# ch4r10t33r/zigz

Hardware: AMD Instinct MI355X
Metric: trace steps/sec proved (BabyBear, 2^20 RV64I trace) (higher is better)
Workload: dtype u32

## Files before the change

zigz_amd/csrc/host_hash.hpp:

```cpp
#pragma once
#include <stddef.h>
#include <stdint.h>

namespace zk {

class Sha3_256 {
  public:
    Sha3_256() { reset(); }
    void reset();
    void update(const uint8_t *data, size_t len);
    void update_le64(uint64_t v);
    void digest_copy(uint8_t out[32]) const;
    void finalize(uint8_t out[32]);
    uint64_t *raw_state() { return st_; }
    size_t *raw_pos() { return &pos_; }

  private:
    uint64_t st_[25];
    size_t pos_;
};

class Transcript {
  public:
    void append_bytes(const uint8_t *d, size_t n) { h_.update(d, n); }
    void append_field(uint64_t canonical) { h_.update_le64(canonical); }
    uint64_t challenge();
    void append_tagged_counter(const uint8_t *tag, size_t tag_len, uint64_t start, uint64_t count);

  private:
    Sha3_256 h_;
};

void sha3_256(const uint8_t *data, size_t len, uint8_t out[32]);
const char *host_keccak_impl();
void host_keccak_permute(uint64_t st[25], int which);
void sha256(const uint8_t *data, size_t len, uint8_t out[32]);

void host_sponge_servers(int n);
bool host_sponge_batching();
bool host_sponge_absorb_tagged(uint64_t st[25], size_t *pos, const uint8_t *tag, size_t tag_len, uint64_t start, uint64_t count);
void host_keccak_permute_x8(uint64_t st[25][8]);

}
```

zigz_amd/csrc/host_sponge_batch.cpp:

```cpp
#include <immintrin.h>
#include <stdint.h>
#include <stdlib.h>
#include <string.h>

#include <algorithm>
#include <atomic>
#include <condition_variable>
#include <deque>
#include <mutex>
#include <thread>
#include <vector>

#include "field.hpp"
#include "host_hash.hpp"

namespace zk {

bool cpu_has_avx512f();

namespace {

constexpr int SLOTS = 8;
constexpr size_t RATE = 136;

const uint64_t RC8[24] = {
    0x0000000000000001ull, 0x0000000000008082ull, 0x800000000000808aull, 0x8000000080008000ull, 0x000000000000808bull,
    0x0000000080000001ull, 0x8000000080008081ull, 0x8000000000008009ull, 0x000000000000008aull, 0x0000000000000088ull,
    0x0000000080008009ull, 0x000000008000000aull, 0x000000008000808bull, 0x800000000000008bull, 0x8000000000008089ull,
    0x8000000000008003ull, 0x8000000000008002ull, 0x8000000000000080ull, 0x000000000000800aull, 0x800000008000000aull,
    0x8000000080008081ull, 0x8000000000008080ull, 0x0000000080000001ull, 0x8000000080008008ull};

__attribute__((target("avx512f"))) void keccak_f1600_x8(uint64_t st[25][SLOTS]) {
#define X8_X3(a, b, c) _mm512_ternarylogic_epi64((a), (b), (c), 0x96)
#define X8_CHI(a, b, c) _mm512_ternarylogic_epi64((a), (b), (c), 0xD2)
#define X8_ROL(a, n) _mm512_rol_epi64((a), (n))
#define X8_B(n, a, cm, rp) X8_ROL(X8_X3(a, cm, rp), n)
#define X8_LD(i) _mm512_load_si512(st[i])
    __m512i a0 = X8_LD(0), a1 = X8_LD(1), a2 = X8_LD(2), a3 = X8_LD(3), a4 = X8_LD(4), a5 = X8_LD(5), a6 = X8_LD(6), a7 = X8_LD(7);
    __m512i a8 = X8_LD(8), a9 = X8_LD(9), a10 = X8_LD(10), a11 = X8_LD(11), a12 = X8_LD(12), a13 = X8_LD(13), a14 = X8_LD(14);
    __m512i a15 = X8_LD(15), a16 = X8_LD(16), a17 = X8_LD(17), a18 = X8_LD(18), a19 = X8_LD(19), a20 = X8_LD(20), a21 = X8_LD(21);
    __m512i a22 = X8_LD(22), a23 = X8_LD(23), a24 = X8_LD(24);
#pragma unroll 2
    for (int r = 0; r < 24; r++) {
        const __m512i c0 = X8_X3(X8_X3(a0, a5, a10), a15, a20), c1 = X8_X3(X8_X3(a1, a6, a11), a16, a21);
        const __m512i c2 = X8_X3(X8_X3(a2, a7, a12), a17, a22), c3 = X8_X3(X8_X3(a3, a8, a13), a18, a23);
        const __m512i c4 = X8_X3(X8_X3(a4, a9, a14), a19, a24);
        const __m512i r0 = X8_ROL(c0, 1), r1 = X8_ROL(c1, 1), r2 = X8_ROL(c2, 1), r3 = X8_ROL(c3, 1), r4 = X8_ROL(c4, 1);
        const __m512i b00 = X8_X3(a0, c4, r1);
        const __m512i b10 = X8_B(1, a1, c0, r2), b20 = X8_B(62, a2, c1, r3), b05 = X8_B(28, a3, c2, r4), b15 = X8_B(27, a4, c3, r0);
        const __m512i b16 = X8_B(36, a5, c4, r1), b01 = X8_B(44, a6, c0, r2), b11 = X8_B(6, a7, c1, r3), b21 = X8_B(55, a8, c2, r4);
        const __m512i b06 = X8_B(20, a9, c3, r0), b07 = X8_B(3, a10, c4, r1), b17 = X8_B(10, a11, c0, r2), b02 = X8_B(43, a12, c1, r3);
        const __m512i b12 = X8_B(25, a13, c2, r4), b22 = X8_B(39, a14, c3, r0), b23 = X8_B(41, a15, c4, r1), b08 = X8_B(45, a16, c0, r2);
        const __m512i b18 = X8_B(15, a17, c1, r3), b03 = X8_B(21, a18, c2, r4), b13 = X8_B(8, a19, c3, r0), b14 = X8_B(18, a20, c4, r1);
        const __m512i b24 = X8_B(2, a21, c0, r2), b09 = X8_B(61, a22, c1, r3), b19 = X8_B(56, a23, c2, r4), b04 = X8_B(14, a24, c3, r0);
        a0 = _mm512_xor_si512(X8_CHI(b00, b01, b02), _mm512_set1_epi64((long long)RC8[r]));
        a1 = X8_CHI(b01, b02, b03); a2 = X8_CHI(b02, b03, b04); a3 = X8_CHI(b03, b04, b00); a4 = X8_CHI(b04, b00, b01);
        a5 = X8_CHI(b05, b06, b07); a6 = X8_CHI(b06, b07, b08); a7 = X8_CHI(b07, b08, b09); a8 = X8_CHI(b08, b09, b05);
        a9 = X8_CHI(b09, b05, b06); a10 = X8_CHI(b10, b11, b12); a11 = X8_CHI(b11, b12, b13); a12 = X8_CHI(b12, b13, b14);
        a13 = X8_CHI(b13, b14, b10); a14 = X8_CHI(b14, b10, b11); a15 = X8_CHI(b15, b16, b17); a16 = X8_CHI(b16, b17, b18);
        a17 = X8_CHI(b17, b18, b19); a18 = X8_CHI(b18, b19, b15); a19 = X8_CHI(b19, b15, b16); a20 = X8_CHI(b20, b21, b22);
        a21 = X8_CHI(b21, b22, b23); a22 = X8_CHI(b22, b23, b24); a23 = X8_CHI(b23, b24, b20); a24 = X8_CHI(b24, b20, b21);
    }
#define X8_ST(i, v) _mm512_store_si512(st[i], (v))
    X8_ST(0, a0); X8_ST(1, a1); X8_ST(2, a2); X8_ST(3, a3); X8_ST(4, a4); X8_ST(5, a5); X8_ST(6, a6); X8_ST(7, a7); X8_ST(8, a8);
    X8_ST(9, a9); X8_ST(10, a10); X8_ST(11, a11); X8_ST(12, a12); X8_ST(13, a13); X8_ST(14, a14); X8_ST(15, a15); X8_ST(16, a16);
    X8_ST(17, a17); X8_ST(18, a18); X8_ST(19, a19); X8_ST(20, a20); X8_ST(21, a21); X8_ST(22, a22); X8_ST(23, a23); X8_ST(24, a24);
}

struct Job {
    uint64_t *st;
    size_t *pos;
    const uint8_t *tag;
    size_t tag_len;
    uint64_t start, count;
    std::mutex m;
    std::condition_variable cv;
    bool done = false;
};

struct Stream {
    static constexpr size_t CHUNK_RECORDS = 272;
    Job *job = nullptr;
    uint64_t v = 0, left = 0;
    size_t rec = 0, rd = 0, wr = 0;
    uint8_t tmpl[32];
    std::vector<uint8_t> buf;

    void open(Job *j) {
        job = j;
        rec = j->tag_len + 8;
        v = j->start % (uint64_t)P;
        left = j->count;
        rd = wr = 0;
        memset(tmpl, 0, sizeof(tmpl));
        memcpy(tmpl, j->tag, j->tag_len < 24 ? j->tag_len : 24);
        buf.resize(CHUNK_RECORDS * rec + RATE + 64);
    }
    size_t avail() const { return wr - rd; }
    bool exhausted() const { return left == 0 && rd == wr; }
    void fill() {
        if (avail() >= RATE || left == 0) return;
        if (rd) {
            memmove(buf.data(), buf.data() + rd, wr - rd);
            wr -= rd;
            rd = 0;
        }
        size_t m = (buf.size() - wr - 32) / rec;
        if (m > left) m = (size_t)left;
        uint8_t *q = buf.data() + wr;
        const size_t tl = job->tag_len;
        if (tl <= 24) {
            for (size_t k = 0; k < m; k++, q += rec) {
                memcpy(q, tmpl, 32);
                memcpy(q + tl, &v, 8);
                if (++v == (uint64_t)P) v = 0;
            }
        } else {
            for (size_t k = 0; k < m; k++, q += rec) {
                memcpy(q, job->tag, tl);
                memcpy(q + tl, &v, 8);
                if (++v == (uint64_t)P) v = 0;
            }
        }
        wr += m * rec;
        left -= m;
    }
};

class Service {
  public:
    ~Service() { resize(0); }

    void resize(int n) {
        std::unique_lock<std::mutex> lk(m_);
        if (n < 0) n = 0;
        if (n > 0 && !cpu_has_avx512f()) n = 0;
        if ((int)threads_.size() == n) return;
        enabled_.store(false, std::memory_order_release);
        stop_ = true;
        cv_.notify_all();
        std::vector<std::thread> old;
        old.swap(threads_);
        lk.unlock();
        for (auto &t : old) t.join();
        lk.lock();
        stop_ = false;
        for (int i = 0; i < n; i++) threads_.emplace_back([this] { serve(); });
        enabled_.store(n > 0, std::memory_order_release);
    }
    bool enabled() const { return enabled_.load(std::memory_order_acquire); }

    bool run(Job &j) {
        {
            std::lock_guard<std::mutex> lk(m_);
            if (threads_.empty() || stop_) return false;
            queue_.push_back(&j);
            pending_.fetch_add(1, std::memory_order_release);
        }
        cv_.notify_one();
        std::unique_lock<std::mutex> lk(j.m);
        j.cv.wait(lk, [&] { return j.done; });
        return true;
    }

  private:
    void serve() {
        alignas(64) uint64_t S[25][SLOTS];
        memset(S, 0, sizeof(S));
        Stream slot[SLOTS];
        size_t pos[SLOTS] = {0};
        int active = 0;
        for (;;) {
            if (active == 0 || (active < SLOTS && pending_.load(std::memory_order_acquire) > 0)) {
                std::unique_lock<std::mutex> lk(m_);
                if (active == 0) cv_.wait(lk, [&] { return stop_ || !queue_.empty(); });
                if (stop_ && active == 0 && queue_.empty()) return;
                for (int s = 0; s < SLOTS && !queue_.empty(); s++) {
                    if (slot[s].job) continue;
                    Job *j = queue_.front();
                    queue_.pop_front();
                    pending_.fetch_sub(1, std::memory_order_relaxed);
                    slot[s].open(j);
                    pos[s] = *j->pos;
                    for (int w = 0; w < 25; w++) S[w][s] = j->st[w];
                    active++;
                }
            }
            if (active == 1 && pending_.load(std::memory_order_acquire) == 0) {
                int s = 0;
                while (!slot[s].job) s++;
                Stream &st = slot[s];
                if (pos[s] == 0) {
                    uint64_t one[25];
                    for (int w = 0; w < 25; w++) one[w] = S[w][s];
                    for (int k = 0; k < 64; k++) {
                        st.fill();
                        if (st.avail() < RATE) break;
                        const uint8_t *src = st.buf.data() + st.rd;
                        for (int w = 0; w < 17; w++) {
                            uint64_t x;
                            memcpy(&x, src + 8 * w, 8);
                            one[w] ^= x;
                        }
                        st.rd += RATE;
                        host_keccak_permute(one, 0);
                    }
                    for (int w = 0; w < 25; w++) S[w][s] = one[w];
                }
            }
            bool permute = false;
            for (int s = 0; s < SLOTS; s++) {
                Stream &st = slot[s];
                if (!st.job) continue;
                st.fill();
                const size_t need = RATE - pos[s];
                size_t n = st.avail() < need ? st.avail() : need;
                const uint8_t *src = st.buf.data() + st.rd;
                if (pos[s] == 0 && n == RATE) {
                    for (int w = 0; w < 17; w++) {
                        uint64_t x;
                        memcpy(&x, src + 8 * w, 8);
                        S[w][s] ^= x;
                    }
                } else if (n) {
                    uint8_t blk[RATE] = {0};
                    memcpy(blk + pos[s], src, n);
                    for (int w = 0; w < 17; w++) {
                        uint64_t x;
                        memcpy(&x, blk + 8 * w, 8);
                        S[w][s] ^= x;
                    }
                }
                st.rd += n;
                pos[s] += n;
                if (pos[s] == RATE) {
                    pos[s] = 0;
                    permute = true;
                } else {
                    retire(S, s, slot, pos);
                    active--;
                }
            }
            if (permute) keccak_f1600_x8(S);
            for (int s = 0; s < SLOTS; s++)
                if (slot[s].job && slot[s].exhausted() && pos[s] == 0) {
                    retire(S, s, slot, pos);
                    active--;
                }
        }
    }

    static void retire(uint64_t S[25][SLOTS], int s, Stream *slot, size_t *pos) {
        Job *j = slot[s].job;
        for (int w = 0; w < 25; w++) j->st[w] = S[w][s];
        *j->pos = pos[s];
        slot[s].job = nullptr;
        std::lock_guard<std::mutex> lk(j->m);
        j->done = true;
        j->cv.notify_one();
    }

    std::mutex m_;
    std::condition_variable cv_;
    std::deque<Job *> queue_;
    std::vector<std::thread> threads_;
    bool stop_ = false;
    std::atomic<int> pending_{0};
    std::atomic<bool> enabled_{false};
};

Service &service() {
    static Service s;
    return s;
}

}

void host_sponge_servers(int n) { service().resize(n); }
bool host_sponge_batching() { return service().enabled(); }

bool host_sponge_absorb_tagged(uint64_t st[25], size_t *pos, const uint8_t *tag, size_t tag_len, uint64_t start, uint64_t count) {
    Job j;
    j.st = st;
    j.pos = pos;
    j.tag = tag;
    j.tag_len = tag_len;
    j.start = start;
    j.count = count;
    return service().run(j);
}

void host_keccak_permute_x8(uint64_t st[25][8]) { keccak_f1600_x8(st); }

void flat_commit_batch(const uint32_t *const *ev, const size_t *n, size_t count, uint8_t (*out)[32]) {
    constexpr size_t WORDS = RATE / 8;
    auto one = [&](size_t i) {
        Sha3_256 h;
        for (size_t j = 0; j < n[i]; j++) h.update_le64(ev[i][j]);
        h.finalize(out[i]);
    };
    std::vector<std::thread> th;
    if (!cpu_has_avx512f()) {
        th.reserve(count);
        for (size_t i = 0; i < count; i++) th.emplace_back(one, i);
        for (auto &t : th) t.join();
        return;
    }
    std::vector<size_t> order(count);
    for (size_t i = 0; i < count; i++) order[i] = i;
    std::sort(order.begin(), order.end(), [&](size_t a, size_t b) { return n[a] > n[b]; });
    auto group = [&](size_t g0) {
        const size_t ns = count - g0 < (size_t)SLOTS ? count - g0 : (size_t)SLOTS;
        alignas(64) uint64_t st[25][SLOTS];
        memset(st, 0, sizeof(st));
        size_t full[SLOTS] = {0};
        size_t blocks = 0;
        for (size_t s = 0; s < ns; s++) {
            full[s] = n[order[g0 + s]] / WORDS;
            if (full[s] > blocks) blocks = full[s];
        }
        auto finish = [&](size_t s) {
            const size_t i = order[g0 + s];
            Sha3_256 h;
            for (int l = 0; l < 25; l++) h.raw_state()[l] = st[l][s];
            *h.raw_pos() = 0;
            for (size_t j = full[s] * WORDS; j < n[i]; j++) h.update_le64(ev[i][j]);
            h.finalize(out[i]);
        };
        for (size_t s = 0; s < ns; s++)
            if (full[s] == 0) finish(s);
        for (size_t b = 0; b < blocks; b++) {
            for (size_t s = 0; s < ns; s++) {
                if (b >= full[s]) continue;
                const uint32_t *v = ev[order[g0 + s]] + b * WORDS;
                for (size_t w = 0; w < WORDS; w++) st[w][s] ^= v[w];
            }
            keccak_f1600_x8(st);
            for (size_t s = 0; s < ns; s++)
                if (full[s] == b + 1) finish(s);
        }
    };
    const size_t groups = (count + SLOTS - 1) / SLOTS;
    th.reserve(groups);
    for (size_t g = 1; g < groups; g++) th.emplace_back(group, g * SLOTS);
    group(0);
    for (auto &t : th) t.join();
}

}
```

Measured before the change: 2.195 billion.

## Generate sponge blocks periodically and fuse 8-lane absorb into Keccak x8

Adds a SpongeBlocks generator that exploits the periodicity of tagged counter records: a buffer of RATE records spans exactly rec blocks, and it is advanced by bumping counters instead of re-serializing each record. The batched server now takes whole blocks per slot and, when all slots have full blocks, absorbs them with an AVX-512 transpose fused into the x8 Keccak permutation instead of scalar per-slot XORs. Partial blocks and stream tails fall back to the old stream path through a seek. The change adds considerable bookkeeping complexity and risk around counter wraparound and block alignment.

```diff
diff --git a/zigz_amd/csrc/host_hash.hpp b/zigz_amd/csrc/host_hash.hpp
--- a/zigz_amd/csrc/host_hash.hpp
+++ b/zigz_amd/csrc/host_hash.hpp
@@ -40,5 +40,6 @@
 bool host_sponge_batching();
 bool host_sponge_absorb_tagged(uint64_t st[25], size_t *pos, const uint8_t *tag, size_t tag_len, uint64_t start, uint64_t count);
 void host_keccak_permute_x8(uint64_t st[25][8]);
+void keccak_f1600_x8_absorb(uint64_t st[25][8], const uint8_t *const blk[8]);
 
 }
diff --git a/zigz_amd/csrc/host_sponge_batch.cpp b/zigz_amd/csrc/host_sponge_batch.cpp
--- a/zigz_amd/csrc/host_sponge_batch.cpp
+++ b/zigz_amd/csrc/host_sponge_batch.cpp
@@ -13,6 +13,7 @@
 
 #include "field.hpp"
 #include "host_hash.hpp"
+#include "sponge_blocks.hpp"
 
 namespace zk {
 
@@ -30,16 +31,50 @@
     0x8000000000008003ull, 0x8000000000008002ull, 0x8000000000000080ull, 0x000000000000800aull, 0x800000008000000aull,
     0x8000000080008081ull, 0x8000000000008080ull, 0x0000000080000001ull, 0x8000000080008008ull};
 
-__attribute__((target("avx512f"))) void keccak_f1600_x8(uint64_t st[25][SLOTS]) {
 #define X8_X3(a, b, c) _mm512_ternarylogic_epi64((a), (b), (c), 0x96)
 #define X8_CHI(a, b, c) _mm512_ternarylogic_epi64((a), (b), (c), 0xD2)
 #define X8_ROL(a, n) _mm512_rol_epi64((a), (n))
 #define X8_B(n, a, cm, rp) X8_ROL(X8_X3(a, cm, rp), n)
 #define X8_LD(i) _mm512_load_si512(st[i])
+#define X8_ST(i, v) _mm512_store_si512(st[i], (v))
+#define X8_ABSORB8(off, r0, r1, r2, r3, r4, r5, r6, r7)                                                                        \
+    {                                                                                                                          \
+        const __m512i x0 = _mm512_loadu_si512(blk[0] + (off)), x1 = _mm512_loadu_si512(blk[1] + (off));                        \
+        const __m512i x2 = _mm512_loadu_si512(blk[2] + (off)), x3 = _mm512_loadu_si512(blk[3] + (off));                        \
+        const __m512i x4 = _mm512_loadu_si512(blk[4] + (off)), x5 = _mm512_loadu_si512(blk[5] + (off));                        \
+        const __m512i x6 = _mm512_loadu_si512(blk[6] + (off)), x7 = _mm512_loadu_si512(blk[7] + (off));                        \
+        const __m512i e01 = _mm512_unpacklo_epi64(x0, x1), o01 = _mm512_unpackhi_epi64(x0, x1);                                \
+        const __m512i e23 = _mm512_unpacklo_epi64(x2, x3), o23 = _mm512_unpackhi_epi64(x2, x3);                                \
+        const __m512i e45 = _mm512_unpacklo_epi64(x4, x5), o45 = _mm512_unpackhi_epi64(x4, x5);                                \
+        const __m512i e67 = _mm512_unpacklo_epi64(x6, x7), o67 = _mm512_unpackhi_epi64(x6, x7);                                \
+        const __m512i ea = _mm512_shuffle_i64x2(e01, e23, 0x88), eb = _mm512_shuffle_i64x2(e01, e23, 0xDD);                    \
+        const __m512i ec = _mm512_shuffle_i64x2(e45, e67, 0x88), ed = _mm512_shuffle_i64x2(e45, e67, 0xDD);                    \
+        const __m512i oa = _mm512_shuffle_i64x2(o01, o23, 0x88), ob = _mm512_shuffle_i64x2(o01, o23, 0xDD);                    \
+        const __m512i oc = _mm512_shuffle_i64x2(o45, o67, 0x88), od = _mm512_shuffle_i64x2(o45, o67, 0xDD);                    \
+        r0 = _mm512_xor_si512(r0, _mm512_shuffle_i64x2(ea, ec, 0x88));                                                         \
+        r1 = _mm512_xor_si512(r1, _mm512_shuffle_i64x2(oa, oc, 0x88));                                                         \
+        r2 = _mm512_xor_si512(r2, _mm512_shuffle_i64x2(eb, ed, 0x88));                                                         \
+        r3 = _mm512_xor_si512(r3, _mm512_shuffle_i64x2(ob, od, 0x88));                                                         \
+        r4 = _mm512_xor_si512(r4, _mm512_shuffle_i64x2(ea, ec, 0xDD));                                                         \
+        r5 = _mm512_xor_si512(r5, _mm512_shuffle_i64x2(oa, oc, 0xDD));                                                         \
+        r6 = _mm512_xor_si512(r6, _mm512_shuffle_i64x2(eb, ed, 0xDD));                                                         \
+        r7 = _mm512_xor_si512(r7, _mm512_shuffle_i64x2(ob, od, 0xDD));                                                         \
+    }
+
+template <bool ABSORB>
+__attribute__((target("avx512f"))) inline void keccak_x8(uint64_t st[25][SLOTS], const uint8_t *const *blk) {
     __m512i a0 = X8_LD(0), a1 = X8_LD(1), a2 = X8_LD(2), a3 = X8_LD(3), a4 = X8_LD(4), a5 = X8_LD(5), a6 = X8_LD(6), a7 = X8_LD(7);
     __m512i a8 = X8_LD(8), a9 = X8_LD(9), a10 = X8_LD(10), a11 = X8_LD(11), a12 = X8_LD(12), a13 = X8_LD(13), a14 = X8_LD(14);
     __m512i a15 = X8_LD(15), a16 = X8_LD(16), a17 = X8_LD(17), a18 = X8_LD(18), a19 = X8_LD(19), a20 = X8_LD(20), a21 = X8_LD(21);
     __m512i a22 = X8_LD(22), a23 = X8_LD(23), a24 = X8_LD(24);
+    if constexpr (ABSORB) {
+        X8_ABSORB8(0, a0, a1, a2, a3, a4, a5, a6, a7)
+        X8_ABSORB8(64, a8, a9, a10, a11, a12, a13, a14, a15)
+        uint64_t w[SLOTS];
+        for (int s = 0; s < SLOTS; s++) memcpy(&w[s], blk[s] + 128, 8);
+        a16 = _mm512_xor_si512(a16, _mm512_set_epi64((long long)w[7], (long long)w[6], (long long)w[5], (long long)w[4],
+                                                     (long long)w[3], (long long)w[2], (long long)w[1], (long long)w[0]));
+    }
 #pragma unroll 2
     for (int r = 0; r < 24; r++) {
         const __m512i c0 = X8_X3(X8_X3(a0, a5, a10), a15, a20), c1 = X8_X3(X8_X3(a1, a6, a11), a16, a21);
@@ -61,11 +96,14 @@
         a17 = X8_CHI(b17, b18, b19); a18 = X8_CHI(b18, b19, b15); a19 = X8_CHI(b19, b15, b16); a20 = X8_CHI(b20, b21, b22);
         a21 = X8_CHI(b21, b22, b23); a22 = X8_CHI(b22, b23, b24); a23 = X8_CHI(b23, b24, b20); a24 = X8_CHI(b24, b20, b21);
     }
-#define X8_ST(i, v) _mm512_store_si512(st[i], (v))
     X8_ST(0, a0); X8_ST(1, a1); X8_ST(2, a2); X8_ST(3, a3); X8_ST(4, a4); X8_ST(5, a5); X8_ST(6, a6); X8_ST(7, a7); X8_ST(8, a8);
     X8_ST(9, a9); X8_ST(10, a10); X8_ST(11, a11); X8_ST(12, a12); X8_ST(13, a13); X8_ST(14, a14); X8_ST(15, a15); X8_ST(16, a16);
     X8_ST(17, a17); X8_ST(18, a18); X8_ST(19, a19); X8_ST(20, a20); X8_ST(21, a21); X8_ST(22, a22); X8_ST(23, a23); X8_ST(24, a24);
 }
+
+__attribute__((target("avx512f"))) void keccak_f1600_x8(uint64_t st[25][SLOTS]) { keccak_x8<false>(st, nullptr); }
+
+alignas(64) const uint8_t ZERO_BLOCK[RATE] = {0};
 
 struct Job {
     uint64_t *st;
@@ -89,12 +127,20 @@
     void open(Job *j) {
         job = j;
         rec = j->tag_len + 8;
-        v = j->start % (uint64_t)P;
-        left = j->count;
-        rd = wr = 0;
         memset(tmpl, 0, sizeof(tmpl));
         memcpy(tmpl, j->tag, j->tag_len < 24 ? j->tag_len : 24);
         buf.resize(CHUNK_RECORDS * rec + RATE + 64);
+        seek(0);
+    }
+    void seek(uint64_t at) {
+        const uint64_t k = at / rec;
+        v = (job->start % (uint64_t)P + k % (uint64_t)P) % (uint64_t)P;
+        left = job->count - k;
+        rd = wr = 0;
+        if (at % rec) {
+            fill();
+            rd = (size_t)(at % rec);
+        }
     }
     size_t avail() const { return wr - rd; }
     bool exhausted() const { return left == 0 && rd == wr; }
@@ -164,11 +210,51 @@
     }
 
   private:
+    struct Slot {
+        Stream st;
+        SpongeBlocks blocks;
+        bool due = false;
+        bool fast = false;
+        uint64_t taken = 0;
+        size_t pos = 0;
+    };
+
+    static const uint8_t *whole_block(Slot &sl) {
+        if (sl.pos != 0) return nullptr;
+        if (sl.due) {
+            const Job *j = sl.st.job;
+            sl.blocks.open(j->tag, j->tag_len, j->start, j->count, sl.taken);
+            sl.due = false;
+            sl.fast = sl.blocks.blocks_left() > 0;
+        }
+        if (sl.fast) {
+            const uint8_t *b = sl.blocks.next();
+            if (sl.blocks.blocks_left() == 0) {
+                sl.fast = false;
+                sl.st.seek(sl.blocks.reached());
+            }
+            return b;
+        }
+        sl.st.fill();
+        if (sl.st.avail() < RATE) return nullptr;
+        const uint8_t *b = sl.st.buf.data() + sl.st.rd;
+        sl.st.rd += RATE;
+        return b;
+    }
+
+    static void absorb_scalar(uint64_t S[25][SLOTS], int s, const uint8_t *blk) {
+        for (int w = 0; w < 17; w++) {
+            uint64_t x;
+            memcpy(&x, blk + 8 * w, 8);
+            S[w][s] ^= x;
+        }
+    }
+
     void serve() {
         alignas(64) uint64_t S[25][SLOTS];
         memset(S, 0, sizeof(S));
-        Stream slot[SLOTS];
-        size_t pos[SLOTS] = {0};
+        std::vector<Slot> slots(SLOTS);
+        Slot *slot = slots.data();
         int active = 0;
         for (;;) {
             if (active == 0 || (active < SLOTS && pending_.load(std::memory_order_acquire) > 0)) {
@@ -176,85 +262,93 @@
                 if (active == 0) cv_.wait(lk, [&] { return stop_ || !queue_.empty(); });
                 if (stop_ && active == 0 && queue_.empty()) return;
                 for (int s = 0; s < SLOTS && !queue_.empty(); s++) {
-                    if (slot[s].job) continue;
+                    if (slot[s].st.job) continue;
                     Job *j = queue_.front();
                     queue_.pop_front();
                     pending_.fetch_sub(1, std::memory_order_relaxed);
-                    slot[s].open(j);
-                    pos[s] = *j->pos;
+                    slot[s].st.open(j);
+                    slot[s].due = SpongeBlocks::serves(j->tag_len);
+                    slot[s].fast = false;
+                    slot[s].taken = 0;
+                    slot[s].pos = *j->pos;
                     for (int w = 0; w < 25; w++) S[w][s] = j->st[w];
                     active++;
                 }
             }
             if (active == 1 && pending_.load(std::memory_order_acquire) == 0) {
                 int s = 0;
-                while (!slot[s].job) s++;
-                Stream &st = slot[s];
-                if (pos[s] == 0) {
+                while (!slot[s].st.job) s++;
+                if (slot[s].pos == 0) {
                     uint64_t one[25];
                     for (int w = 0; w < 25; w++) one[w] = S[w][s];
                     for (int k = 0; k < 64; k++) {
-                        st.fill();
-                        if (st.avail() < RATE) break;
-                        const uint8_t *src = st.buf.data() + st.rd;
+                        const uint8_t *src = whole_block(slot[s]);
+                        if (!src) break;
                         for (int w = 0; w < 17; w++) {
                             uint64_t x;
                             memcpy(&x, src + 8 * w, 8);
                             one[w] ^= x;
                         }
-                        st.rd += RATE;
                         host_keccak_permute(one, 0);
                     }
                     for (int w = 0; w < 25; w++) S[w][s] = one[w];
                 }
             }
-            bool permute = false;
+            const uint8_t *blk[SLOTS];
+            bool all_whole = true;
             for (int s = 0; s < SLOTS; s++) {
-                Stream &st = slot[s];
-                if (!st.job) continue;
-                st.fill();
-                const size_t need = RATE - pos[s];
-                size_t n = st.avail() < need ? st.avail() : need;
-                const uint8_t *src = st.buf.data() + st.rd;
-                if (pos[s] == 0 && n == RATE) {
-                    for (int w = 0; w < 17; w++) {
-                        uint64_t x;
-                        memcpy(&x, src + 8 * w, 8);
-                        S[w][s] ^= x;
+                blk[s] = ZERO_BLOCK;
+                if (!slot[s].st.job) continue;
+                blk[s] = whole_block(slot[s]);
+                if (!blk[s]) all_whole = false;
+            }
+            if (all_whole) {
+                keccak_f1600_x8_absorb(S, blk);
+            } else {
+                bool permute = false;
+                for (int s = 0; s < SLOTS; s++) {
+                    Slot &sl = slot[s];
+                    Stream &st = sl.st;
+                    if (!st.job) continue;
+                    if (blk[s]) {
+                        absorb_scalar(S, s, blk[s]);
+                        permute = true;
+                        continue;
                     }
-                } else if (n) {
-                    uint8_t blk[RATE] = {0};
-                    memcpy(blk + pos[s], src, n);
-                    for (int w = 0; w < 17; w++) {
-                        uint64_t x;
-                        memcpy(&x, blk + 8 * w, 8);
-                        S[w][s] ^= x;
+                    st.fill();
+                    const size_t need = RATE - sl.pos;
+                    size_t n = st.avail() < need ? st.avail() : need;
+                    if (n) {
+                        uint8_t part[RATE] = {0};
+                        memcpy(part + sl.pos, st.buf.data() + st.rd, n);
+                        absorb_scalar(S, s, part);
+                    }
+                    st.rd += n;
+                    sl.taken += n;
+                    sl.pos += n;
+                    if (sl.pos == RATE) {
+                        sl.pos = 0;
+                        permute = true;
+                    } else {
+                        retire(S, s, slot);
+                        active--;
                     }
                 }
-                st.rd += n;
-                pos[s] += n;
-                if (pos[s] == RATE) {
-                    pos[s] = 0;
-                    permute = true;
-                } else {
-                    retire(S, s, slot, pos);
+                if (permute) keccak_f1600_x8(S);
+            }
+            for (int s = 0; s < SLOTS; s++)
+                if (slot[s].st.job && slot[s].pos == 0 && !slot[s].due && !slot[s].fast && slot[s].st.exhausted()) {
+                    retire(S, s, slot);
                     active--;
                 }
-            }
-            if (permute) keccak_f1600_x8(S);
-            for (int s = 0; s < SLOTS; s++)
-                if (slot[s].job && slot[s].exhausted() && pos[s] == 0) {
-                    retire(S, s, slot, pos);
-                    active--;
-                }
-        }
-    }
-
-    static void retire(uint64_t S[25][SLOTS], int s, Stream *slot, size_t *pos) {
-        Job *j = slot[s].job;
+        }
+    }
+
+    static void retire(uint64_t S[25][SLOTS], int s, Slot *slot) {
+        Job *j = slot[s].st.job;
         for (int w = 0; w < 25; w++) j->st[w] = S[w][s];
-        *j->pos = pos[s];
-        slot[s].job = nullptr;
+        *j->pos = slot[s].pos;
+        slot[s].st.job = nullptr;
         std::lock_guard<std::mutex> lk(j->m);
         j->done = true;
         j->cv.notify_one();
@@ -291,6 +385,9 @@
 }
 
 void host_keccak_permute_x8(uint64_t st[25][8]) { keccak_f1600_x8(st); }
+__attribute__((target("avx512f"))) void keccak_f1600_x8_absorb(uint64_t st[25][8], const uint8_t *const blk[8]) {
+    keccak_x8<true>(st, blk);
+}
 
 void flat_commit_batch(const uint32_t *const *ev, const size_t *n, size_t count, uint8_t (*out)[32]) {
     constexpr size_t WORDS = RATE / 8;
diff --git a/zigz_amd/csrc/sponge_blocks.hpp b/zigz_amd/csrc/sponge_blocks.hpp
--- /dev/null
+++ b/zigz_amd/csrc/sponge_blocks.hpp
@@ -0,0 +1,90 @@
+#pragma once
+#include <stddef.h>
+#include <stdint.h>
+#include <string.h>
+
+#include "field.hpp"
+
+namespace zk {
+
+class SpongeBlocks {
+  public:
+    static constexpr size_t RATE = 136;
+    static constexpr size_t MAX_REC = 40;
+    static bool serves(size_t tag_len) { return tag_len + 8 <= MAX_REC; }
+
+    void open(const uint8_t *tag, size_t tag_len, uint64_t start, uint64_t count, uint64_t offset) {
+        tag_len_ = tag_len;
+        rec_ = tag_len + 8;
+        memset(tmpl_, 0, sizeof(tmpl_));
+        memcpy(tmpl_, tag, tag_len);
+        const uint64_t total = count * rec_;
+        left_ = total >= offset ? (total - offset) / RATE : 0;
+        reached_ = offset;
+        cut_ = (size_t)(offset % rec_);
+        first_ = (start % (uint64_t)P + (offset / rec_) % (uint64_t)P) % (uint64_t)P;
+        bi_ = 0;
+        if (left_) regenerate();
+    }
+    uint64_t blocks_left() const { return left_; }
+    uint64_t reached() const { return reached_; }
+    const uint8_t *next() {
+        if (bi_ == rec_) {
+            next_period();
+            bi_ = 0;
+        }
+        left_--;
+        reached_ += RATE;
+        return buf_ + RATE * bi_++;
+    }
+
+  private:
+    static bool crosses(uint64_t first) { return first + RATE >= (uint64_t)P; }
+
+    void put(uint8_t *dst, uint64_t v, size_t a, size_t b) const {
+        uint8_t r[MAX_REC];
+        memcpy(r, tmpl_, tag_len_);
+        memcpy(r + tag_len_, &v, 8);
+        memcpy(dst, r + a, b - a);
+    }
+    void put_cut_records() {
+        if (!cut_) return;
+        put(buf_, first_, cut_, rec_);
+        uint64_t v = first_ + RATE;
+        if (v >= (uint64_t)P) v -= (uint64_t)P;
+        put(buf_ + RATE * rec_ - cut_, v, 0, cut_);
+    }
+    void regenerate() {
+        put_cut_records();
+        uint64_t v = first_;
+        for (size_t k = 0; k < RATE; k++) {
+            if (k || !cut_) put(buf_ + (k * rec_ - cut_), v, 0, rec_);
+            if (++v == (uint64_t)P) v = 0;
+        }
+    }
+    void next_period() {
+        const bool crossed = crosses(first_);
+        first_ += RATE;
+        if (first_ >= (uint64_t)P) first_ -= (uint64_t)P;
+        if (crossed || crosses(first_)) {
+            regenerate();
+            return;
+        }
+        for (size_t k = cut_ ? 1 : 0; k < RATE; k++) {
+            uint8_t *q = buf_ + (k * rec_ - cut_ + tag_len_);
+            uint32_t c;
+            memcpy(&c, q, 4);
+            c += (uint32_t)RATE;
+            memcpy(q, &c, 4);
+        }
+        put_cut_records();
+    }
+
+    alignas(64) uint8_t buf_[RATE * MAX_REC];
+    uint8_t tmpl_[MAX_REC];
+    size_t tag_len_ = 0, rec_ = 8, cut_ = 0, bi_ = 0;
+    uint64_t first_ = 0;
+    uint64_t left_ = 0, reached_ = 0;
+};
+
+}
```

Measured after the change: 2.189 billion. Within noise of the previous version (-0.3%).
